# RemyMuj/UnityRayTracer

Measured on AMD Instinct MI355X. Metric: Mrays/sec @1920x1080, 8 bounces, higher is better.
Workload: dtype f32

## Files before the change

### unityraytracer_amd/csrc/context.cpp

```cpp
#include "experiments.h"
#include "context_impl.h"

#include <climits>
#include <limits>
#include <memory>

#include "normals.h"
#include "normals_plan.h"
#include "present.h"
#include "reproject.h"
#include "skin.h"

using namespace urtd;

namespace {

const char* const kBindNames[B_COUNT] = {"_MeshObjects", "_Vertices", "_Indices", "_Normals", "_Spheres", "_MeshBVH", "_SphereBVH"};
const int kBindStride[B_COUNT] = {URT_STRIDE_MESHOBJECT, URT_STRIDE_VEC3, URT_STRIDE_INDEX, URT_STRIDE_VEC3,
                                  URT_STRIDE_SPHERE, URT_STRIDE_BVHNODE, URT_STRIDE_BVHNODE};

std::string g_create_error;

BlasResult g_debug_blas;

// ... 821 lines not shown
  if (!device_src || !hip_stream) return fail(ctx, URT_ERR_INVALID_ARGUMENT, "device_src / hip_stream is NULL");
  Texture* t = find_texture(ctx, texture);
  if (!t) return fail(ctx, URT_ERR_INVALID_HANDLE, "unknown texture handle");
  if (first_group_row < 0 || row_stride < 1) return fail(ctx, URT_ERR_INVALID_ARGUMENT, "bad strip arguments");
  if (ctx->pend.n > 0) {
    bool touched = ctx->pend.tex == texture;
    for (const PostOp& q : ctx->pend.ops) touched = touched || q.touches(texture);
    if (touched) { int rc = flush_pending(ctx); if (rc) return rc; }
  }
  if (in_slab(ctx, *t)) { int rc = detach_from_slab(ctx, *t); if (rc) return rc; }
  int n_strips = strip_count((t->h + 7) / 8, first_group_row, row_stride);
  t->other_writes = true;
  URT_HIP(ctx, hipSetDevice(ctx->device));
  if (rgb) URT_HIP(ctx, launch_pack_rows_rgb(t->dev, (float*)const_cast<void*>(device_src), t->w, t->h, first_group_row, row_stride, n_strips, false,
                                            alpha, (hipStream_t)hip_stream));
  else URT_HIP(ctx, launch_pack_rows(t->dev, (float4*)const_cast<void*>(device_src), t->w, t->h, first_group_row, row_stride, n_strips, false,
                                     (hipStream_t)hip_stream));
  return URT_OK;
}

int urt_texture_unpack_rows_on(urt_context* ctx, urt_handle texture, int first_group_row, int row_stride, const void* device_src,
                               void* hip_stream) {
  return unpack_on_impl(ctx, texture, first_group_row, row_stride, device_src, hip_stream, false, 0.0f);
}

int urt_texture_pack_rows_rgb(urt_context* ctx, urt_handle texture, int first_group_row, int row_stride, void* device_dst,
                              uint64_t* out_bytes) {
  return pack_impl(ctx, texture, first_group_row, row_stride, device_dst, true, out_bytes, true);
}

int urt_texture_unpack_rows_rgb(urt_context* ctx, urt_handle texture, int first_group_row, int row_stride, const void* device_src,
                                float alpha, void* hip_stream) {
  if (ctx && !device_src) return fail(ctx, URT_ERR_INVALID_ARGUMENT, "device_src is NULL");
  if (hip_stream) return unpack_on_impl(ctx, texture, first_group_row, row_stride, device_src, hip_stream, true, alpha);
  return pack_impl(ctx, texture, first_group_row, row_stride, const_cast<void*>(device_src), false, nullptr, true, alpha);
}

int urt_texture_unpack_rows(urt_context* ctx, urt_handle texture, int first_group_row, int row_stride, const void* device_src) {
  if (ctx && !device_src) return fail(ctx, URT_ERR_INVALID_ARGUMENT, "device_src is NULL");
  return pack_impl(ctx, texture, first_group_row, row_stride, const_cast<void*>(device_src), false, nullptr);
}

namespace {
enum : unsigned { kBool = 1, kStale = 2, kFlushAgain = 4, kOnChange = 8 };
struct OptionRow { const char* name; int urt_context::Options::* field; int lo, hi; const char* msg; unsigned flags; bool (*ok)(int); };
using O = urt_context::Options;
const OptionRow kOptions[] = {
  {"blas_builder", &O::blas_builder, -1, 3, "blas_builder must be -1 (auto), 0 (host SAH), 1 (GPU LBVH), 2 (GPU LBVH built top-down within a depth budget) or 3 (binned SAH on the GPU)", kStale | kOnChange, nullptr},
  {"frames_per_launch", &O::frames_per_launch, 0, kMaxFramesPerLaunch, "frames_per_launch must be in [0, 64] (0 = auto)", 0, nullptr},
  {"count_stats", &O::count_stats, INT_MIN, INT_MAX, "", kBool, nullptr},
  {"time_dispatch", &O::time_dispatch, INT_MIN, INT_MAX, "", kBool, nullptr},
  {"kernel_mode", &O::kernel_mode, 0, 5, "kernel_mode must be 0..5", 0, nullptr},
  {"block_threads", &O::block_threads, 64, 256, "block_threads must be 64, 128 or 256", 0, [](int v) { return v == 64 || v == 128 || v == 256; }},
  {"blas_leaf_max", nullptr , 1, 8, "blas_leaf_max must be in [1, 8]", kStale, nullptr},
  {"blas_min", &O::blas_min, 0, 256, "blas_min must be in [0, 256] (0 = auto; kernel_mode 5 counts the waiting rays of a workgroup)", 0, nullptr},
  {"blas_exit", &O::blas_exit, 0, 64, "blas_exit must be in [0, 64] (0 = auto)", 0, nullptr},
  {"refill_min", &O::refill_min, 1, 64, "refill_min must be in [1, 64]", 0, nullptr},
  {"waves_per_cu", &O::waves_per_cu, 0, 32, "waves_per_cu must be in [0, 32] (0 = auto)", 0, nullptr},
  {"sched_block", &O::sched_block, 0, 256, "sched_block must be 0 (auto), 64 or 256", 0, [](int v) { return v == 0 || v == 64 || v == 256; }},
  {"stack_pad", &O::stack_pad, 0, 96, "stack_pad must be in [0, 96]", 0, nullptr},
  {"radiance_persist", &O::radiance_persist, -1, 1, "radiance_persist must be -1 (auto), 0 or 1", 0, nullptr},
  {"shade_min", &O::shade_min, 1, 64, "shade_min must be in [1, 64]", 0, nullptr},
  {"front_list", &O::front_list, -1, 2, "front_list must be -1 (auto), 0, 1 or 2", 0, nullptr},
  {"shade_split", &O::shade_split, -1, 1, "shade_split must be -1 (auto), 0 or 1", 0, nullptr},
  {"serve_refill", &O::serve_refill, 1, 64, "serve_refill must be in [1, 64]", 0, nullptr},
  {"sky_min", &O::sky_min, 1, 64, "sky_min must be in [1, 64]", 0, nullptr},
  {"tile_order", &O::tile_order, -1, 1, "tile_order must be -1 (auto), 0 or 1", 0, nullptr},
  {"lds_tlas", &O::lds_tlas, INT_MIN, INT_MAX, "", kBool, nullptr},
  {"top_front", &O::top_front, -1, 1, "top_front must be -1 (auto), 0 or 1", 0, nullptr},
  {"top_nodes", &O::top_nodes, -1, kTopOrderNodes, "top_nodes must be in [0, 256], or -1 (auto)", 0, nullptr},
  {"pool_k", &O::pool_k, 1, 4, "pool_k must be in [1, 4]", 0, nullptr},
  {"pool_refill", &O::pool_refill, 1, 256, "pool_refill must be in [1, 256]", 0, nullptr},
  {"pool_blas_min", &O::pool_blas_min, 1, 256, "pool_blas_min must be in [1, 256]", 0, nullptr},
  {"pool_blas_exit", &O::pool_blas_exit, 1, 64, "pool_blas_exit must be in [1, 64]", 0, nullptr},
  {"pool_other_min", &O::pool_other_min, 1, 64, "pool_other_min must be in [1, 64]", 0, nullptr},
  {"pool_inloop", &O::pool_inloop, 1, 64, "pool_inloop must be in [1, 64]", 0, nullptr},
  {"frame_group", &O::frame_group, 1, kMaxFramesPerLaunch, "frame_group must be in [1, 64]", 0, nullptr},
  {"work_shards", &O::work_shards, 1, (int)kWorkShards, "work_shards must be a power of two in [1, 64]", 0, [](int v) { return (v & (v - 1)) == 0; }},
  {"qnodes", &O::qnodes, -1, 1, "qnodes must be -1 (auto), 0 or 1", kStale, nullptr},
  {"lbvh_slack", &O::lbvh_slack, 0, 16, "lbvh_slack must be 0..16", kStale | kOnChange, nullptr},
  {"overlap_launches", &O::overlap_launches, 0, 2, "overlap_launches must be 0 (off), 1 (auto) or 2 (always)", kFlushAgain, nullptr},
  {"blas_cones", &O::blas_cones, -1, 1, "blas_cones must be -1 (auto), 0 or 1", kStale | kOnChange, nullptr},
  {"front_cull", &O::front_cull, 0, 1, "front_cull must be 0 or 1", kFlushAgain | kStale | kOnChange, nullptr},
  {"refit", &O::refit, INT_MIN, INT_MAX, "", kBool | kStale, nullptr},
  {"refit_vertices", &O::refit_vertices, INT_MIN, INT_MAX, "", kBool, nullptr},
  {"refit_rebuild_pct", &O::refit_rebuild_pct, 0, INT_MAX, "refit_rebuild_pct must be 0 (never rebuild) or greater than 100", 0, [](int v) { return v == 0 || v > 100; }},
  {"watchdog_cap", &O::watchdog_cap, 0, INT_MAX, "watchdog_cap must be >= 0 (0 = auto)", 0, nullptr},
  {"xcd_run", &O::xcd_run, 0, 4096, "xcd_run must be in [0, 4096] (0 = auto)", 0, nullptr},
};
}

int urt_set_option(urt_context* ctx, const char* name, int value) {
  if (!ctx) return fail(nullptr, URT_ERR_INVALID_ARGUMENT, "ctx is NULL");
  if (!name) return fail(ctx, URT_ERR_INVALID_ARGUMENT, "option name is NULL");
  { (void)hipSetDevice(ctx->device); int rc = flush_pending(ctx); if (rc) return rc; }
  const OptionRow* r = std::find_if(std::begin(kOptions), std::end(kOptions), [&](const OptionRow& o) { return std::strcmp(name, o.name) == 0; });
  if (r == std::end(kOptions)) return fail(ctx, URT_ERR_INVALID_ARGUMENT, std::string("unknown option ") + name);
  if (value < r->lo || value > r->hi || (r->ok && !r->ok(value))) return fail(ctx, URT_ERR_INVALID_ARGUMENT, r->msg);
  if (r->flags & kBool) value = value ? 1 : 0;
  const bool act = !(r->flags & kOnChange) || ctx->opt.*r->field != value;
  if ((r->flags & kFlushAgain) && act) { int rc = flush_pending(ctx); if (rc) return rc; }
  if ((r->flags & kStale) && act) { ctx->scene_dirty = true; ctx->dirty_full = true; }
  if (r->field) ctx->opt.*r->field = value; else set_blas_leaf_max(value);
  return URT_OK;
}

int urt_get_counters(urt_context* ctx, urt_counters* out) {
  if (!ctx) return fail(nullptr, URT_ERR_INVALID_ARGUMENT, "ctx is NULL");
  if (!out) return fail(ctx, URT_ERR_INVALID_ARGUMENT, "out is NULL");
  URT_HIP(ctx, hipSetDevice(ctx->device));
  { int rc = flush_pending(ctx); if (rc) return rc; }
  URT_HIP(ctx, hipStreamSynchronize(touch(ctx)));
  resolve_timing(ctx);
  std::vector<DevCounters> shards(kCounterShards);
  URT_HIP(ctx, hipMemcpy(shards.data(), ctx->d_counters.get(), sizeof(DevCounters) * kCounterShards, hipMemcpyDeviceToHost));
  std::memset(out, 0, sizeof *out);
  for (const DevCounters& dc : shards) {
    out->rays += dc.rays; out->tlas_nodes += dc.tlas_nodes; out->blas_nodes += dc.blas_nodes; out->tri_tests += dc.tri_tests;
    out->sphere_tests += dc.sphere_tests; out->hit_tri += dc.hit_tri; out->hit_sphere += dc.hit_sphere;
    out->hit_ground += dc.hit_ground; out->hit_sky += dc.hit_sky;
    out->watchdog_trips += (uint32_t)dc.watchdog;
  }
  out->pixels = ctx->pixels_dispatched;
  out->dispatches = ctx->dispatches;
  out->launches = ctx->launches;
  out->trace_ms = ctx->trace_ms;
  return URT_OK;
}

int urt_reset_counters(urt_context* ctx) {
  if (!ctx) return fail(nullptr, URT_ERR_INVALID_ARGUMENT, "ctx is NULL");
  URT_HIP(ctx, hipSetDevice(ctx->device));
  { int rc = flush_pending(ctx); if (rc) return rc; }
  URT_HIP(ctx, hipStreamSynchronize(touch(ctx)));
  resolve_timing(ctx);
  URT_HIP(ctx, hipMemset(ctx->d_counters.get(), 0, sizeof(DevCounters) * kCounterShards));
  if (ctx->h_trip_flag) __atomic_store_n(ctx->h_trip_flag.get(), 0u, __ATOMIC_RELEASE);
  ctx->dispatches = 0;
  ctx->launches = 0;
  ctx->pixels_dispatched = 0;
  ctx->trace_ms = 0;
  return URT_OK;
}

#ifdef URT_STAMPS
__attribute__((visibility("default"))) int urt_debug_read_stamps(urt_context* ctx, unsigned long long* out, int n_waves) {
  (void)hipStreamSynchronize(touch(ctx));
  hipError_t e = hipMemcpy(out, (char*)ctx->d_next.get() + urt_context::kStampOffset, (size_t)n_waves * sizeof(unsigned long long), hipMemcpyDeviceToHost);
  (void)hipMemset((char*)ctx->d_next.get() + urt_context::kStampOffset, 0, urt_context::kStampBytes);
  return (int)e;
}
#endif

int urt_debug_serve_stats(urt_context* ctx, unsigned long long* out6) {
  if (!ctx) return fail(nullptr, URT_ERR_INVALID_ARGUMENT, "ctx is NULL");
  if (!out6) return fail(ctx, URT_ERR_INVALID_ARGUMENT, "out6 is NULL");
  URT_HIP(ctx, hipSetDevice(ctx->device));
  { int rc = flush_pending(ctx); if (rc) return rc; }
  URT_HIP(ctx, hipStreamSynchronize(touch(ctx)));
  std::vector<DevCounters> shards(kCounterShards);
  URT_HIP(ctx, hipMemcpy(shards.data(), ctx->d_counters.get(), sizeof(DevCounters) * kCounterShards, hipMemcpyDeviceToHost));
  for (int q = 0; q < 6; q++) out6[q] = 0;
  for (const DevCounters& dc : shards) for (int q = 0; q < 6; q++) out6[q] += dc.serve[q];
  return URT_OK;
}

// ... 172 lines not shown
```

### unityraytracer_amd/csrc/context_impl.h

```cpp
#pragma once
#include <hip/hip_runtime.h>

#include <algorithm>
#include <cmath>
#include <cstdio>
#include <cstring>
#include <new>
#include <string>
#include <unordered_map>
#include <utility>
#include <vector>

#include "../../include/urt.h"
#include "../../include/urt_math.h"
#include "blas_builder.h"
#include "kernels.h"
#include "owned.h"
#include "urt_device.h"

namespace urtd {

struct Buffer {
  int count = 0, stride = 0;
  std::vector<uint8_t> host;
  bool has_data = false;
  int dirty_first = 0, dirty_last = -1;
  void mark_dirty(int first, int last) {
    if (dirty_last < dirty_first) { dirty_first = first; dirty_last = last; }
    else { dirty_first = std::min(dirty_first, first); dirty_last = std::max(dirty_last, last); }
  }
  DeviceBuf<char> mirror;
  int stale_first = 0, stale_last = -1;
  uint64_t downloads = 0;
  bool stale() const { return stale_last >= stale_first; }
  void mark_stale(int first, int last) {
    if (!stale()) { stale_first = first; stale_last = last; }
    else { stale_first = std::min(stale_first, first); stale_last = std::max(stale_last, last); }
  }
};

struct Texture {
  int w = 0, h = 0;
  float4* dev = nullptr;
  float4* own = nullptr;
  DeviceBuf<float4> storage;
  bool external = false;
  bool ptr_exposed = false;
  bool other_writes = false;
  int n_regions = 0;
  int rg[4] = {0, 0, 0, 0};
};

struct DevNormalsPlan {
  urt_handle vertices = 0;
  int n_vertices = 0;
  int first = 0, count = 0, n_lists = 0, n_triangles = 0, n_entries = 0, max_valence = 0;
  DeviceBuf<int32_t> tris, entries, ranges;
  uint64_t device_bytes = 0;
};

enum BindSlot { B_MESHOBJECTS, B_VERTICES, B_INDICES, B_NORMALS, B_SPHERES, B_MESHBVH, B_SPHEREBVH, B_COUNT };

}

struct urt_context {
  urtd::Stream own_stream;
  int device = 0;
  hipStream_t stream = nullptr;
  std::string err;
  std::unordered_map<urt_handle, urtd::Buffer> buffers;
  std::unordered_map<urt_handle, urtd::Texture> textures;
  std::unordered_map<urt_handle, urtd::DevNormalsPlan> normals_plans;
  urt_handle next_id = 1;

  urt_handle bound[urtd::B_COUNT] = {0, 0, 0, 0, 0, 0, 0};
  urt_handle t_sky = 0, t_result = 0;
  float c2w[16] = {0}, invp[16] = {0};
  bool c2w_set = false, invp_set = false;
  float pixel_off[2] = {0, 0};
  float seed = 0;
  int num_bounces = 0, num_rays = 0;

  struct Options {
    int refit = 1;
    int refit_vertices = 1;
    int refit_rebuild_pct = 0;
    int qnodes = 0;
    int count_stats = 0, time_dispatch = 0, kernel_mode = 3;
    int block_threads = 64, xcd_run = 0 , work_shards = 64, frame_group = 64, refill_min = 16, waves_per_cu = 0 , blas_min = 0 , blas_exit = 0 ;
    int pool_k = 2, pool_refill = 32, pool_blas_min = 48, pool_blas_exit = 8, pool_inloop = 16, pool_other_min = 24;
    int sched_block = 0;
    int stack_pad = 0;
    int radiance_persist = -1;
    int shade_min = 32, sky_min = 32;
    int serve_refill = 16;
    int front_list = -1;
    int shade_split = -1;
    int tile_order = -1;
    int lds_tlas = 1;
    int top_front = -1;
    int top_nodes = -1;
    int blas_builder = -1;
    int frames_per_launch = 0;
    int watchdog_cap = 0;
    int lbvh_slack = 6;
    int front_cull = 1;
    int overlap_launches = 1;
    int blas_cones = -1;
  } opt;

  bool scene_dirty = true;
  unsigned int dirty_slots = 0;
  bool dirty_full = true;
  struct Scene {
    urtd::DevScene ds{};
    std::vector<urtd::DeviceBuf<char>> scene_allocs;
    struct RefitAux {
      const float* vertices = nullptr; const int32_t* indices = nullptr;
      const float* normals = nullptr;
      int32_t* renormed = nullptr;
      double* cost_base = nullptr; double* cost_now = nullptr;
      int32_t* parent = nullptr; int32_t* node_mesh = nullptr; int32_t* depth = nullptr;
      float4* cbox = nullptr; unsigned int* ext = nullptr;
      float* matrices = nullptr; int32_t* moved = nullptr;
      bool ready = false;
    } refit;
    float4* qbuf = nullptr;
    float4* cbuf = nullptr;
    float qnode_quality = 0;
    int4* cone_rng[2] = {nullptr, nullptr};
    const int4* cone_ranges = nullptr;
    bool cones_in_use = false;
    const float4* aov_albedo = nullptr;
    size_t cap_materials = 0, cap_mesh_tlas = 0, cap_sphere_tlas = 0, cap_sphere_pr = 0, cap_aov_albedo = 0;
    int32_t* d_mesh_leaf = nullptr;
    size_t cap_mesh_leaf = 0;
    int walk_f4 = 0;
    int n_blas_nodes = 0;
    int n_scene_tris = 0;
    int scene_max_depth = 0;
    int tlas_stack = 2, blas_stack = 2;
    unsigned int watchdog_steps = 1u << 16;
    std::vector<int32_t> h_mesh_root, h_small_first;
    std::vector<int32_t> h_vert_lo, h_vert_hi;
    int n_vertices = 0, n_normals = 0;
    std::vector<float> h_cost_base;
    std::vector<uint8_t> prev_mesh_objects;
  } scene;
  uint64_t scene_epoch = 0;
  float last_prepare_ms = 0;
  int last_builder = 0;
  uint64_t refitted_meshes = 0, incremental_preps = 0;
  uint64_t deformed_meshes = 0, renormed_meshes = 0, deform_bytes = 0, forced_rebuilds = 0;
  float last_cost_ratio = 0;
  urtd::BlasCache blas_cache;
  int sched_groups = 0;
  urtd::DeviceBuf<float4> zero_sky;

  urtd::PathQueues q{};
  urtd::DeviceBuf<float4> q_store[2][4];
  urtd::DeviceBuf<unsigned int> q_counts;

  urtd::DeviceBuf<urtd::DevCounters> d_counters;
  static constexpr size_t kStampOffset = urtd::kWorkShards * 128, kStampBytes = 65536 * 16 * sizeof(unsigned long long), kWorkCounterBytes = kStampOffset + kStampBytes;
  urtd::DeviceBuf<unsigned int> d_next;
  urtd::DeviceBuf<float4> d_mail;
  static constexpr int kTableSlots = 4;
  urtd::PinnedBuf<urtd::FrameUniforms> h_tables; urtd::DeviceBuf<urtd::FrameUniforms> d_tables;
  urtd::Event table_ev[kTableSlots];
  unsigned int table_next = 0;
  uint64_t pixels_dispatched = 0;
  int n_cus = 256;

  uint64_t dispatches = 0;
  std::vector<std::pair<urtd::Event, urtd::Event>> timing;
  float trace_ms = 0;

  enum class OpKind { BlendAdd, BlendHistory, Copy, PackRows };
  struct PostOp {
    OpKind kind;
// ... 140 lines not shown
```

### unityraytracer_amd/csrc/frame_batch.cpp

```cpp
#include "experiments.h"
#include "context_impl.h"

#include "reproject.h"

namespace urtd {

static unsigned int sched_trip_cap(urt_context* ctx, const FrameParams& P, int n_frames) {
  if (ctx->opt.watchdog_cap > 0) return (unsigned int)ctx->opt.watchdog_cap;
  uint64_t per = std::max<uint64_t>(1, (uint64_t)std::max(1, P.num_rays) * (uint64_t)std::max(1, P.num_bounces) / 8u);
  uint64_t cap = (1ull << 24) * (uint64_t)std::max(1, n_frames) * per;
  return (unsigned int)std::min<uint64_t>(cap, 0xfffffff0ull);
}

static int ensure_queues(urt_context* ctx, size_t n_paths, size_t n_counts) {
  for (int k = 0; k < 8; k++) {
    if (int rc = reserve(ctx, ctx->q_store[k / 4][k % 4], n_paths, "path queue allocation", touch(ctx))) return rc;
    ctx->q.s[k / 4][k % 4] = ctx->q_store[k / 4][k % 4].get();
  }
  if (int rc = reserve(ctx, ctx->q_counts, n_counts, "path queue allocation", touch(ctx))) return rc;
  ctx->q.counts = ctx->q_counts.get();
  return URT_OK;
}

int resolve_timing(urt_context* ctx) {
// ... 336 lines not shown
    if (ctx->stream != ctx->own_stream.get()) return 1;
    uint64_t frame_bytes = (uint64_t)P.width * (uint64_t)P.height * sizeof(float4);
    lim = (int)std::min<uint64_t>(kAutoFrames, std::max<uint64_t>(1, (8ull << 30) / std::max<uint64_t>(1, frame_bytes)));
  }
  uint64_t slots = std::max<uint64_t>(1, ((uint64_t)P.tiles_x * (uint64_t)P.n_strips + (uint64_t)std::max(64, ctx->opt.xcd_run)) * 64u);
  lim = (int)std::min<uint64_t>((uint64_t)lim, std::max<uint64_t>(1, 0xfffffffeull / slots / 2));
  return std::max(1, std::min(lim, (int)kMaxFramesPerLaunch));
}

int bind_sky(urt_context* ctx, DevScene& S) {
  Texture* sky = find_texture(ctx, ctx->t_sky);
  if (sky) { S.sky = sky->dev; S.sky_w = sky->w; S.sky_h = sky->h; }
  else {
    if (!ctx->zero_sky) {
      URT_HIP(ctx, ctx->zero_sky.alloc(1));
      URT_HIP(ctx, hipMemsetAsync(ctx->zero_sky.get(), 0, sizeof(float4), touch(ctx)));
    }
    S.sky = ctx->zero_sky.get(); S.sky_w = 1; S.sky_h = 1;
  }
  return URT_OK;
}

int do_dispatch(urt_context* ctx, int kernel, int gx, int gy, int gz, int first_row, int row_stride) {
  if (kernel != 0) return fail(ctx, URT_ERR_INVALID_ARGUMENT, "kernel index must be 0 (CSMain)");
  if (gx < 0 || gy < 0 || gz < 0 || first_row < 0 || row_stride < 1)
    return fail(ctx, URT_ERR_INVALID_ARGUMENT, "negative thread-group count or bad strip arguments");
  urt_handle res_h = ctx->t_result;
  Texture* res = find_texture(ctx, res_h);
  if (!res) return fail(ctx, URT_ERR_UNBOUND, "Dispatch: no texture bound to \"Result\" (RM:803)");
  if (res->w > 65535 || res->h > 65535) return fail(ctx, URT_ERR_INVALID_ARGUMENT, "Result larger than 65535 pixels per side");
  URT_HIP(ctx, hipSetDevice(ctx->device));
  if (int rc = current_scene(ctx)) return rc;
  ctx->dispatches++;
  if (gx == 0 || gy == 0 || gz == 0) return URT_OK;

  DevScene S = ctx->scene.ds;
  { int rc = bind_sky(ctx, S); if (rc) return rc; }

  FrameParams P{};
  std::memcpy(P.c2w, ctx->c2w, sizeof P.c2w);
  std::memcpy(P.invp, ctx->invp, sizeof P.invp);
  P.pixel_off_x = ctx->pixel_off[0]; P.pixel_off_y = ctx->pixel_off[1];
  P.seed = ctx->seed;
  P.num_bounces = ctx->num_bounces; P.num_rays = ctx->num_rays;
  P.width = res->w; P.height = res->h;
  long rw = std::min<long>((long)gx * 8, res->w), rh = std::min<long>((long)gy * 8, res->h);
  P.region_w = (int)rw; P.region_h = (int)rh;
  P.tiles_x = (P.region_w + 7) / 8;
  P.first_group_row = first_row; P.row_stride = row_stride;
  P.n_strips = strip_count((P.region_h + 7) / 8, first_row, row_stride);
  P.tlas_stack = lane_stack_size(ctx).tlas; P.blas_stack = lane_stack_size(ctx).blas; P.watchdog_steps = ctx->scene.watchdog_steps;
  P.block_threads = ctx->opt.block_threads; P.xcd_run = ctx->opt.xcd_run; P.tile_order = ctx->opt.tile_order >= 0 ? ctx->opt.tile_order : (S.n_meshes == 0 ? 1 : 0); P.refill_min = ctx->opt.refill_min;
  P.blas_min = ctx->opt.blas_min > 0 ? ctx->opt.blas_min : (S.n_meshes > 1 ? 24 : 16);
  P.blas_exit = ctx->opt.blas_exit > 0 ? ctx->opt.blas_exit : (S.n_meshes > 1 ? 9 : 14); P.shade_min = ctx->opt.shade_min; P.sky_min = ctx->opt.sky_min;
  P.n_frames = 1; P.frame_stride = 0;
  P.sched_trips = sched_trip_cap(ctx, P, 1); P.trip_flag = ctx->d_trip_flag;
  if (P.n_strips == 0 || P.tiles_x == 0) return URT_OK;
  P.n_shards = ctx->opt.work_shards; P.frame_group = ctx->opt.frame_group;
  if (ctx->opt.xcd_run <= 0) P.xcd_run = ctx->opt.kernel_mode >= 2 ? auto_run_length(P, 1) : 1;
  if ((uint64_t)P.tiles_x * (uint64_t)P.n_strips * 64u >= 0xffffffffull)
    return fail(ctx, URT_ERR_INVALID_ARGUMENT, "Dispatch: too many pixel slots in one dispatch");

  {
    uint64_t px = 0;
    for (int j = 0; j < P.n_strips; j++) {
      int y0 = (first_row + j * row_stride) * 8;
      px += (uint64_t)std::max(0, std::min(P.region_h - y0, 8)) * (uint64_t)P.region_w;
    }
    ctx->pixels_dispatched += px;
  }
  bool degenerate = P.num_bounces <= 0 || P.num_rays <= 0;
  int mode = degenerate ? 0 : ctx->opt.kernel_mode;
  if ((mode == 3 || mode == 5) && P.num_bounces >= (1 << 24)) mode = 2;
  bool count = ctx->opt.count_stats != 0;
  const int region[4] = {P.region_w, P.region_h, first_row, row_stride};
  const bool full_cover = P.region_w == res->w && P.region_h == res->h && first_row == 0 && row_stride == 1;

  if (mode == 3 || mode == 5) {
    bool top_in_front = ctx->opt.top_front < 0 ? S.n_meshes > 1 : ctx->opt.top_front != 0;
    P.serve = mode == 5 && ctx->scene.n_blas_nodes > 0;
    P.pool_inloop = ctx->opt.serve_refill;
    int front_mode = configure_sched(ctx, S, P, top_in_front);
    P.shade_split = ctx->opt.shade_split != 0;
    const FrameUniforms fu = bound_camera(ctx);
    bool same_region = res->n_regions == 1 && std::memcmp(res->rg, region, sizeof region) == 0;
    bool renamable = !res->external && !res->ptr_exposed && (full_cover || (!res->other_writes && (res->n_regions == 0 || same_region)));
    int limit = renamable ? batch_limit(ctx, P) : 1;
    urt_context::Pending& B = ctx->pend;
    if (B.n > 0) {
      const FrameParams& Q = B.P;
      bool same = B.tex == res_h && B.scene_epoch == ctx->scene_epoch && B.S.sky == S.sky && B.S.sky_w == S.sky_w && B.S.sky_h == S.sky_h &&
                  B.count == count && B.front_mode == front_mode && Q.serve == P.serve && Q.num_bounces == P.num_bounces && Q.num_rays == P.num_rays &&
                  Q.width == P.width && Q.height == P.height && Q.region_w == P.region_w && Q.region_h == P.region_h &&
                  Q.first_group_row == P.first_group_row && Q.row_stride == P.row_stride && B.n < B.limit && limit > 1;
      if (!same) { int rc = flush_pending(ctx); if (rc) return rc; }
    }
    if (limit > 1 && B.n == 0) {
      int rc = ensure_slab(ctx, res_h, *res, limit); if (rc) return rc;
      if (!ctx->slab || ctx->slab_tex != res_h || ctx->slab_frames < 2) limit = 1;
    }
    if (B.n == 0) { int rc = bind_sky(ctx, S); if (rc) return rc; }
    if (limit <= 1) {
      FrameTable T{};
      T.f[0] = fu;
      P.frame_group = 1;
      int rc = launch_sched_frames(ctx, S, P, T, res->dev, front_mode, count);
      if (rc) return rc;
    } else {
      if (B.n == 0) {
        B.limit = std::min(limit, ctx->slab_frames);
        B.tex = res_h; B.scene_epoch = ctx->scene_epoch; B.S = S; B.P = P; B.front_mode = front_mode; B.count = count;
      }
      B.T.f[B.n] = fu;
      res->dev = ctx->slab.get() + (size_t)B.n * ctx->slab_stride;
      B.n++;
    }
  } else {
    int rc = flush_pending(ctx); if (rc) return rc;
    int nb = 0, k = 0;
    if (mode == 1) {
      size_t n_paths = (size_t)P.tiles_x * 64 * (size_t)P.n_strips;
      rc = ensure_queues(ctx, n_paths, (size_t)P.num_rays * (size_t)(P.num_bounces + 1));
      if (rc) return rc;
    } else if (mode == 2) {
      int waves_per_block = P.block_threads / 64;
      long want = ((long)P.tiles_x * P.n_strips + waves_per_block - 1) / waves_per_block;
      int wpc = ctx->opt.waves_per_cu;
      if (wpc <= 0) wpc = 20;
      long resident = (long)ctx->n_cus * wpc / waves_per_block;
      nb = (int)std::max(1L, std::min(want, resident));
    } else if (mode == 4) {
      P.block_threads = 64;
      P.refill_min = ctx->opt.pool_refill; P.blas_min = ctx->opt.pool_blas_min; P.blas_exit = ctx->opt.pool_blas_exit;
      P.pool_inloop = ctx->opt.pool_inloop; P.pool_other_min = ctx->opt.pool_other_min;
      k = ctx->opt.pool_k;
      size_t lds = pool_lds_bytes(P, k);
      while (k > 1 && lds > 160 * 1024) { k--; lds = pool_lds_bytes(P, k); }
      if (lds > 160 * 1024) return fail(ctx, URT_ERR_OUT_OF_MEMORY, "kernel_mode 4: the scene's traversal stacks do not fit the LDS of one CU; use kernel_mode 3");
      int fit = (int)std::max<size_t>(1, (160 * 1024) / lds);
      int wpc = ctx->opt.waves_per_cu > 0 ? ctx->opt.waves_per_cu : fit;
      long want = ((long)P.tiles_x * P.n_strips * 64 + 64L * k - 1) / (64L * k);
      nb = (int)std::max(1L, std::min(want, (long)ctx->n_cus * wpc));
    }
    const hipStream_t st = touch(ctx);
    rc = timed_launch(ctx, st, mode, 0, P, count, ctx->opt.waves_per_cu, [&](TraceLaunchRecord* rec) {
      switch (mode) {
        case 1: return launch_wavefront(S, P, ctx->q, res->dev, ctx->d_counters.get(), count, st, rec);
        case 2: return launch_persist(S, P, res->dev, ctx->d_counters.get(), ctx->d_next.get(), nb, count, st, rec);
        case 4: return launch_pool(S, P, res->dev, ctx->d_counters.get(), ctx->d_next.get(), nb, k, count, st, rec);
        default: return launch_mega(S, P, res->dev, ctx->d_counters.get(), count, st, rec);
      }
    });
    if (rc) return rc;
  }
  if (res->n_regions == 0) { res->n_regions = 1; std::memcpy(res->rg, region, sizeof region); }
  else if (std::memcmp(res->rg, region, sizeof region) != 0) res->n_regions = 2;
  return URT_OK;
}

}
```

### unityraytracer_amd/csrc/front_device.h

```cpp
#pragma once
#include "frame_device.h"

namespace {

struct FrontLds {
  const float4* mesh_tlas = nullptr;
  const int32_t* mesh_root = nullptr;
  const float4* sphere_tlas = nullptr;
  const float4* sphere_pr = nullptr;
  const float4* small_tris = nullptr;
  const int32_t* small_first = nullptr;
};

template <bool COUNT, bool TOPF = false, bool RAYS = true, int SP0 = 0, bool CONES = false>
__device__ __forceinline__ bool trace_front(const DevScene& S, bool fresh, v3 o, v3 d, HitRec& best, int& check, bool& seen,
                                            int* tl, int stride, int32_t& cur, LocalCounters& lc, const FrontLds& L = FrontLds(),
                                            const float4* top = nullptr, int top_nodes = 0, int* bl = nullptr, int* sp_out = nullptr) {
  if (fresh) {
    if (RAYS) lc.rays++;
    best.t = URT_INF; best.kid = 0; best.u = 0; best.v = 0;
    float t = -o.y / d.y;
    if (t > 0 && t < best.t) { best.t = t; best.kid = 1; }
    check = 0; seen = false;
    if (S.n_meshes > 0) { check = 1; tl[0] = 0; }
  }
  v3 rcp = mk3(1.0f / (d.x + kEPSILON), 1.0f / (d.y + kEPSILON), 1.0f / (d.z + kEPSILON));
  const bool may_cull = S.cull_any != 0;
  while (check > 0) {
    check--;
    int bi = tl[check * stride];
    bool hit = false; int index = -1;
    float t_min = 0.0f, t_max = 0.0f; int cull_word = 0;
    if (bi < S.n_mesh_tlas) {
      if (COUNT) lc.tlas_nodes++;
      float4 a, b;
      if (L.mesh_tlas) { a = L.mesh_tlas[2 * bi]; b = L.mesh_tlas[2 * bi + 1]; } else { a = S.mesh_tlas[2 * bi]; b = S.mesh_tlas[2 * bi + 1]; }
      index = as_int(a.w);
      if (may_cull) { hit = tlas_slab_t(a, b, o, rcp, t_min, t_max); cull_word = as_int(b.w); }
      else hit = tlas_slab(a, b, o, rcp);
    }
    if (hit) {
      if (index < 0) { tl[check * stride] = bi * 2 + 1; check++; tl[check * stride] = bi * 2 + 2; check++; }
      else seen = true;
    }
    bool culled = false;
    if (cull_word != 0) { float t = -o.y / d.y; culled = tlas_cull(t_min, t_max, t > 0 ? t : URT_INF); }
    if (seen && !culled && index >= 0 && index < S.n_meshes) {
      int32_t root;
      if (L.mesh_root) root = L.mesh_root[index]; else root = S.mesh_root[index];
      if (root < 0 && root != kBlasDone) {
        int bi_local = -1;
        if (L.small_tris) test_leaf<COUNT>(S, root, o, d, best, bi_local, lc, L.small_tris, L.small_first[index]);
        else test_leaf<COUNT>(S, root, o, d, best, bi_local, lc);
      } else if (root != kEmptyMeshRoot) {
        if (TOPF) {
          int sp = SP0;
          if (root < top_nodes) {
            BlasRay R = blas_ray(o, d);
            if (SP0 == 1) root = blas_walk_top_ptr<COUNT, CONES>(top, top_nodes, root, R, best.t, bl, sp, lc, CONES ? cone_ray_word(d) : 0);
            else do root = blas_node_step_top<COUNT>(top, root, R, best.t, bl, sp, lc); while (root >= 0 && root < top_nodes);
          }
          *sp_out = sp;
          if (root == kBlasDone) continue;
        }
        cur = root;
        return true;
      }
    }
  }
  if (S.n_spheres > 0) {
    int c2 = 1; tl[0] = 0; bool seen2 = false;
    while (c2 > 0) {
      c2--;
      int bi = tl[c2 * stride];
      bool hit = false; int index = -1;
      if (bi < S.n_sphere_tlas) {
        if (COUNT) lc.tlas_nodes++;
        float4 a, b;
        if (L.sphere_tlas) { a = L.sphere_tlas[2 * bi]; b = L.sphere_tlas[2 * bi + 1]; } else { a = S.sphere_tlas[2 * bi]; b = S.sphere_tlas[2 * bi + 1]; }
        index = as_int(a.w);
        hit = tlas_slab(a, b, o, rcp);
      }
      if (hit) {
        if (index < 0) { tl[c2 * stride] = bi * 2 + 1; c2++; tl[c2 * stride] = bi * 2 + 2; c2++; }
        else seen2 = true;
      }
      if (seen2 && index >= 0 && index < S.n_spheres) intersect_sphere<COUNT>(S, index, o, d, best, lc, L.sphere_pr);
    }
  }
  return false;
}

__device__ __forceinline__ int list_get(const int* tl, int j) {
  unsigned int w = (unsigned int)tl[j >= 6 ? 64 : 0];
  return (int)((w >> (5 * (j >= 6 ? j - 6 : j))) & 31u);
}

#ifdef URT_STAMPS
#define URT_FS_DECL , unsigned long long* fs
#define URT_FS_ARG , fs_arr
#define URT_FS(stmt) stmt
#else
#define URT_FS_DECL
#define URT_FS_ARG
#define URT_FS(stmt)
#endif
template <bool COUNT, int SP0 = 0, bool CONES = false>
__device__ __forceinline__ int front_listed(const DevScene& S, const FrameParams& P, bool mine, bool fresh, v3 o, v3 d, HitRec& best, int& cs,
                                            int* tl, int32_t& cur, LocalCounters& lc, const FrontLds& L, const float4* top, int* bl, int& sp,
                                            unsigned int& wave_rays URT_FS_DECL) {
  URT_FS(unsigned long long fs_t0 = wall_clock64();)
  int remaining = cs & 0xff, cursor = cs >> 8;
  const int n_fresh = __popcll(wballot(mine && fresh)), n_resumed = __popcll(wballot(mine && !fresh));
  const bool walk_now = n_fresh >= 16 || n_resumed == 0;
  if (!walk_now) mine = mine && !fresh;
  else wave_rays += (unsigned int)n_fresh;
  const bool put_off = !walk_now && fresh;
  if (mine && fresh) {
    best.t = URT_INF; best.kid = 0; best.u = 0; best.v = 0;
    float t = -o.y / d.y;
    if (t > 0 && t < best.t) { best.t = t; best.kid = 1; }
    v3 rcp = mk3(1.0f / (d.x + kEPSILON), 1.0f / (d.y + kEPSILON), 1.0f / (d.z + kEPSILON));
    int count = 0, check = 0;
    unsigned int l0 = 0, l1 = 0;
    bool seen = false;
    if (S.n_meshes > 0) { check = 1; tl[0] = 0; }
    const float t_ground = best.t;
    while (check > 0) {
      check--;
      int bi = tl[check * 64];
      bool hit = false, culled = false; int index = -1;
      if (bi < S.n_mesh_tlas) {
        if (COUNT) lc.tlas_nodes++;
        float4 a = L.mesh_tlas[2 * bi], b = L.mesh_tlas[2 * bi + 1];
        index = as_int(a.w);
        float t_min, t_max;
        hit = tlas_slab_t(a, b, o, rcp, t_min, t_max);
        culled = leaf_culled(b, t_min, t_max, t_ground);
      }
      if (hit) {
        if (index < 0) { tl[check * 64] = bi * 2 + 1; check++; tl[check * 64] = bi * 2 + 2; check++; }
        else seen = true;
      }
      if (seen && !culled && index >= 0 && index < S.n_meshes && L.mesh_root[index] != kEmptyMeshRoot) {
        if (count < 6) l0 |= (unsigned int)index << (5 * count); else l1 |= (unsigned int)index << (5 * (count - 6));
        count++;
      }
    }
    tl[0] = (int)l0; tl[64] = (int)l1;
    remaining = count; cursor = 0;
  }
  URT_FS(if (walk_now && n_fresh > 0) { fs[0] += wall_clock64() - fs_t0; fs[3]++; fs[6] += (unsigned long long)n_fresh; })
  bool need = false;
  bool has = mine && remaining > 0;
  for (;;) {
    int obj = 0; int32_t root = kEmptyMeshRoot;
    URT_FS(unsigned long long fs_t1 = wall_clock64();)
    for (;;) {
      if (has) { obj = list_get(tl, cursor); root = L.mesh_root[obj]; }
      bool small = has && root < 0;
      if (wballot(small) == 0) break;
      URT_FS(fs[4]++;)
      if (small) {
        int bi_local = -1;
        if (L.small_tris) test_leaf<COUNT>(S, root, o, d, best, bi_local, lc, L.small_tris, L.small_first[obj]);
        else test_leaf<COUNT>(S, root, o, d, best, bi_local, lc);
        cursor++; remaining--; has = remaining > 0;
      }
    }
    URT_FS(fs[1] += wall_clock64() - fs_t1; fs_t1 = wall_clock64();)
// ... 166 lines not shown
```

### unityraytracer_amd/csrc/kernels.hip

```cpp
#include "experiments.h"
#include "front_device.h"
#include "launch_host.h"
#include <utility>

namespace {

#ifndef URT_SCHED_OCC
#define URT_SCHED_OCC 5
#endif
template <bool COUNT, int BLOCK, int FMODE, bool MULTI, bool QN = false>
__global__ __launch_bounds__(BLOCK, URT_SCHED_OCC) void k_sched(DevScene S, FrameParams P, const FrameUniforms* __restrict__ T, float4* __restrict__ result, DevCounters* ctr,
                                               unsigned int* __restrict__ next) {
  constexpr bool CONES = !COUNT && !QN;
  extern __shared__ int lds[];
  float4* lds4 = (float4*)lds;
  const float4* top = lds4;
  for (int i = threadIdx.x; i < P.top_nodes * 4; i += blockDim.x) lds4[i] = S.blas_cnodes[i];
  int at = P.top_nodes * 4;
  FrontLds L;
  if (P.lds_mesh) {
    for (int i = threadIdx.x; i < 2 * S.n_mesh_tlas; i += blockDim.x) lds4[at + i] = S.mesh_tlas[i];
    L.mesh_tlas = lds4 + at; at += 2 * S.n_mesh_tlas;
    for (int i = threadIdx.x; i < S.n_meshes; i += blockDim.x) ((int32_t*)(lds4 + at))[i] = S.mesh_root[i];
    L.mesh_root = (const int32_t*)(lds4 + at); at += (S.n_meshes + 3) / 4;
    if (P.lds_small) {
      for (int i = threadIdx.x; i < S.n_meshes; i += blockDim.x) ((int32_t*)(lds4 + at))[i] = S.mesh_small_first[i];
      L.small_first = (const int32_t*)(lds4 + at); at += (S.n_meshes + 3) / 4;
      for (int m = threadIdx.x; m < S.n_meshes; m += blockDim.x) {
        int sf = S.mesh_small_first[m];
        if (sf >= 0) {
          uint32_t code = ~(uint32_t)S.mesh_root[m];
          uint32_t first = code >> 3, cnt = (code & 7u) + 1u;
          for (uint32_t q = 0; q < 3 * cnt; q++) lds4[at + 3 * sf + q] = S.tri_verts[3 * (size_t)first + q];
        }
      }
      L.small_tris = lds4 + at; at += 3 * S.n_small;
    }
  }
  WalkLds W;
  if (FMODE == 3) {
    const float4* wsrc = S.mesh_tlas + 2 * S.n_mesh_tlas;
    for (int i = threadIdx.x; i < P.walk_f4; i += blockDim.x) lds4[at + i] = wsrc[i];
    W.hdr = (const int*)(lds4 + at); W.pos_tab = W.hdr + 16; W.eval = lds4 + at + 20; at += P.walk_f4;
    if (P.lds_small) {
      for (int m = threadIdx.x; m < S.n_meshes; m += blockDim.x) {
        int sf = S.mesh_small_first[m];
        if (sf >= 0) {
          uint32_t code = ~(uint32_t)S.mesh_root[m];
          uint32_t first = code >> 3, cnt = (code & 7u) + 1u;
          for (uint32_t q = 0; q < 3 * cnt; q++) lds4[at + 3 * sf + q] = S.tri_verts[3 * (size_t)first + q];
        }
      }
      L.small_tris = lds4 + at; at += 3 * S.n_small;
    }
  }
  if (P.lds_sphere) {
    for (int i = threadIdx.x; i < 2 * S.n_sphere_tlas; i += blockDim.x) lds4[at + i] = S.sphere_tlas[i];
    L.sphere_tlas = lds4 + at; at += 2 * S.n_sphere_tlas;
    for (int i = threadIdx.x; i < S.n_spheres; i += blockDim.x) lds4[at + i] = S.sphere_pr[i];
    L.sphere_pr = lds4 + at; at += S.n_spheres;
  }
  __syncthreads();
  int* tl = lds + at * 4 + (threadIdx.x >> 6) * ((P.tlas_stack + P.blas_stack) * 64) + (threadIdx.x & 63);
  int* bl = tl + P.tlas_stack * 64;
  LocalCounters lc;
  unsigned int tiles_per_frame;
  const unsigned int ntiles = launch_tiles(P, tiles_per_frame);
  WorkCursor wc; wc.shard = blockIdx.x & ((unsigned int)P.n_shards - 1u);
  bool exhausted = false;
  int st = ST_DEAD;
  int xy = 0;
  int ray_i = 0, kf = 0;
  float seed = 0;
  v3 o = mk3(0, 0, 0), d = mk3(0, 0, 1), energy = mk3(0, 0, 0), res = mk3(0, 0, 0), avg = mk3(0, 0, 0);
  HitRec best; best.t = URT_INF; best.kid = 0; best.u = 0; best.v = 0;
  int cs = 0;
  bl[0] = kBlasDone;
  int32_t cur = kBlasDone; int sp = 1, best_i = -1;
  unsigned int wave_iters = 0, wave_rays = 0;
  bool watchdog = false;
#ifdef URT_STAMPS
  unsigned long long ph_t[4] = {0, 0, 0, 0}, ph_lanes[4] = {0, 0, 0, 0}, ph_trips[4] = {0, 0, 0, 0};
  unsigned long long t_begin = wall_clock64(), t_dry = 0;
  unsigned long long c_begin = __builtin_amdgcn_s_memtime();
  unsigned long long dr_trips[4] = {0, 0, 0, 0}, dr_t[3] = {0, 0, 0}, dr_live = 0, dr_lanes3 = 0;
  unsigned long long fs_arr[7] = {0, 0, 0, 0, 0, 0, 0};
  unsigned long long rf_t[3] = {0, 0, 0};
  unsigned long long bl_part[3] = {0, 0, 0};
#endif

  for (;;) {
    if (watchdog) break;
#ifdef URT_STAMPS
    if (exhausted && !t_dry) t_dry = wall_clock64();
#endif
    unsigned long long mD = wballot(st == ST_DEAD);
    int nD = __popcll(mD);
    int nB = __popcll(wballot(st == ST_BLAS));
    int nS = __popcll(wballot(st == ST_SHADE));
    int nK = __popcll(wballot(st == ST_SKY));
    int nF = __popcll(wballot(st == ST_FRONT || st == ST_RESUME));
    if (!exhausted && nD > 0 && (nD >= P.refill_min || nB + nS + nK + nF == 0)) {
      int x = 0, y = 0, frame = 0;
#ifdef URT_STAMPS
      unsigned long long t_rf = wall_clock64();
#endif
      bool got = wave_fetch_pixels(P, mD, st == ST_DEAD, next, ntiles, wc, exhausted, x, y, tiles_per_frame, &frame);
#ifdef URT_STAMPS
      rf_t[0] += wall_clock64() - t_rf; t_rf = wall_clock64();
#endif
      for_each_frame(got, frame, [&](int f, bool mine) {
        if (mine) {
          st = ST_FRONT;
          ray_i = 0; kf = frame << 24; xy = x | (y << 16);
          avg = mk3(0, 0, 0); res = mk3(0, 0, 0); energy = mk3(1, 1, 1);
          camera_ray_frame(T, f, P, x, y, true, seed, o, d);
        }
      });
#ifdef URT_STAMPS
      rf_t[1] += wall_clock64() - t_rf; rf_t[2]++;
#endif
      nF = __popcll(wballot(st == ST_FRONT || st == ST_RESUME));
      nD = __popcll(wballot(st == ST_DEAD));
    }
    bool can_refill = !exhausted && nD >= P.refill_min;
    if (++wave_iters > P.sched_trips) { watchdog = true; break; }
    int phase;
    int exit_below = 1;
    bool sky_too = false;
    if (nB >= P.blas_min) { phase = ST_BLAS; if (nS + nK + nF > 0 || can_refill) exit_below = min(P.blas_exit, nB); }
    else if (P.shade_split) {
      if (nS >= P.shade_min) phase = ST_SHADE;
      else if (nK >= P.sky_min) phase = ST_SKY;
      else if (nF > 0) phase = ST_FRONT;
      else if (nS > 0 && nS >= nK) phase = ST_SHADE;
      else if (nK > 0) phase = ST_SKY;
      else if (nB > 0) phase = ST_BLAS;
      else if (exhausted) break;
      else continue;
    }
    else if (nS + nK >= P.shade_min) { phase = nS > 0 ? ST_SHADE : ST_SKY; sky_too = true; }
    else if (nF > 0) phase = ST_FRONT;
    else if (nS + nK > 0) { phase = nS > 0 ? ST_SHADE : ST_SKY; sky_too = true; }
    else if (nB > 0) phase = ST_BLAS;
    else if (exhausted) break;
    else continue;

#ifdef URT_STAMPS
    unsigned long long t_ph = wall_clock64();
    int ph_id = phase == ST_FRONT ? 0 : phase == ST_BLAS ? 1 : 2;
    ph_lanes[ph_id] += (unsigned long long)(phase == ST_FRONT ? nF : phase == ST_BLAS ? nB : phase == ST_SHADE ? nS : nK);
    ph_trips[ph_id]++;
    if (exhausted) { if (!dr_live) dr_live = 64 - nD; dr_trips[ph_id]++; }
#endif
    if (phase == ST_FRONT) {
      if (FMODE < 2) wave_rays += (unsigned int)__popcll(wballot(st == ST_FRONT));
      if (FMODE >= 2) {
        bool mine = st == ST_FRONT || st == ST_RESUME;
        int r = FMODE == 3 ? front_masked<COUNT, 1, CONES>(S, P, mine, st == ST_FRONT, o, d, best, cs, tl, cur, lc, L, W, top, bl, sp, wave_rays URT_FS_ARG)
                           : front_listed<COUNT, 1, CONES>(S, P, mine, st == ST_FRONT, o, d, best, cs, tl, cur, lc, L, top, bl, sp, wave_rays URT_FS_ARG);
        if (mine && r != 2) {
          if (r == 1) { best_i = -1; st = ST_BLAS; }
          else st = best.t < URT_INF ? ST_SHADE : ST_SKY;
        }
      } else if (st == ST_FRONT || st == ST_RESUME) {
        sp = 1;
        int check = cs & 0xff; bool seen = (cs >> 8) != 0;
        bool need = FMODE == 1 ? trace_front<COUNT, true, false, 1, CONES>(S, st == ST_FRONT, o, d, best, check, seen, tl, 64, cur, lc, L, top, P.top_nodes, bl, &sp)
                               : trace_front<COUNT, false, false, 1>(S, st == ST_FRONT, o, d, best, check, seen, tl, 64, cur, lc, L);
        cs = check | (seen ? 256 : 0);
        if (need) { best_i = -1; st = ST_BLAS; }
        else st = best.t < URT_INF ? ST_SHADE : ST_SKY;
      }
    } else if (phase == ST_BLAS) {
      bool mine = st == ST_BLAS;
      BlasRay R = blas_ray(o, d);
      int* spp = bl + (sp - 1) * 64;
      const int rw = CONES ? cone_ray_word(d) : 0;
      if (mine && cur >= 0 && cur < P.top_nodes) {
        do {
          if (COUNT) lc.blas_nodes++;
          const float4* n = top + 4 * cur;
          cur = CONES ? blas_node_eval_cone_ptr(n[0], n[1], n[2], n[3], R, best.t, rw, spp) : blas_node_eval_ptr(n[0], n[1], n[2], n[3], R, best.t, spp);
        } while (cur >= 0 && cur < P.top_nodes);
      }
      int32_t c = mine ? cur : kBlasDone;
      int budget = __builtin_amdgcn_readfirstlane((int)min(P.watchdog_steps, 0x7fffffffu));
      const int exit_s = __builtin_amdgcn_readfirstlane(exit_below);
      QRay Q;
      if (QN) Q = make_qray(o, d, S.blas_qnodes[0], S.blas_qnodes[1]);
      for (;;) {
        int nA = __popcll(wballot(c != kBlasDone));
        if (nA < exit_s) break;
        if (--budget < 0) { watchdog = true; break; }
#ifdef URT_STAMPS
        ph_trips[3]++; ph_lanes[3] += (unsigned long long)nA;
        if (exhausted) { dr_trips[3]++; dr_lanes3 += (unsigned long long)nA; }
#endif
        int nI = __popcll(wballot(c >= 0));
        bool node_trip = 2 * nI >= nA;
#ifdef URT_STAMPS
        bl_part[0] += (unsigned long long)(node_trip ? nI : nA - nI); bl_part[1] += node_trip ? 1 : 0; bl_part[2] += (unsigned long long)(node_trip ? nA - nI : 0);
#endif
        if (node_trip) {
          if (QN) {
            if (c >= 0) {
              const float4* n = (const float4*)((const char*)(S.blas_qnodes + 2) + ((uint32_t)c << 5));
              float4 u0 = n[0], u1 = n[1];
              c = qnode_eval_ptr(u0, u1, Q, best.t, spp);
            }
          } else if (c >= 0) {
            if (COUNT) lc.blas_nodes++;
            const float4* n = (const float4*)((const char*)S.blas_cnodes + ((uint32_t)c << 6));
            float4 q0 = n[0], q1 = n[1], q2 = n[2], q3 = n[3];
            c = CONES ? blas_node_eval_cone_ptr(q0, q1, q2, q3, R, best.t, rw, spp) : blas_node_eval_ptr(q0, q1, q2, q3, R, best.t, spp);
          }
        } else if (c < 0 && c != kBlasDone) {
          test_leaf<COUNT>(S, c, o, d, best, best_i, lc);
          c = *spp; spp -= 64;
        }
      }
      if (mine) { cur = c; sp = ((int)(spp - bl) >> 6) + 1; }
      if (mine && cur == kBlasDone) st = ((FMODE == 3 ? cs : (cs & 0xff)) == 0 && S.n_spheres == 0) ? (best.t < URT_INF ? ST_SHADE : ST_SKY) : ST_RESUME;
    } else {
      bool next_ray = false;
      bool cont = false, shaded = false;
      if (phase == ST_SHADE) {
        if (st == ST_SHADE) { shaded = true; cont = shade_surface<COUNT>(S, best, o, d, energy, res, seed, (float)(xy & 0xffff), (float)((unsigned)xy >> 16), lc); }
      }
      if (phase == ST_SKY || (sky_too && nK > 0)) {
        if (st == ST_SKY) { shaded = true; cont = shade_sky<COUNT>(S, d, energy, res, lc); }
      }
      if (shaded) {
        kf++;
        st = ST_FRONT;
        if (!cont || (kf & 0xffffff) >= P.num_bounces) {
          v3 sum = (MULTI ? avg : mk3(0, 0, 0)) + res;
          if (MULTI) { avg = sum; ray_i++; next_ray = ray_i < P.num_rays; }
          if (!next_ray) {
            float n = (float)P.num_rays;
            st_nt(result + (size_t)((unsigned)kf >> 24) * P.frame_stride + (size_t)((unsigned)xy >> 16) * P.width + (xy & 0xffff),
                      MULTI ? make_float4(sum.x / n, sum.y / n, sum.z / n, 1.0f) : make_float4(sum.x, sum.y, sum.z, 1.0f));
            st = ST_DEAD;
          }
        }
      }
      if (MULTI) {
        for_each_frame(next_ray, (int)((unsigned)kf >> 24), [&](int f, bool mine) {
          if (mine) {
            res = mk3(0, 0, 0); energy = mk3(1, 1, 1); kf &= (int)0xff000000;
            camera_ray_frame(T, f, P, xy & 0xffff, (int)((unsigned)xy >> 16), false, seed, o, d);
          }
        });
// ... 183 lines not shown
```

### unityraytracer_amd/csrc/urt_device.h

```cpp
#pragma once
#include <stdint.h>
#include <hip/hip_runtime.h>

#include "blas_builder.h"

namespace urtd {

struct DevScene {
  const float4* mesh_tlas;   int n_mesh_tlas;
  const float4* sphere_tlas; int n_sphere_tlas;
  const float4* sphere_pr;   int n_spheres;
  const float4* materials;
  const int32_t* mesh_root;  int n_meshes;
  const int32_t* mesh_small_first; int n_small;
  const float4* blas_nodes;
  const float4* blas_cnodes;
  const float4* blas_qnodes;
  const float4* tri_verts;
  const float4* tri_norms;
  const float4* sky;         int sky_w, sky_h;
  int cull_any;
};

struct FrameParams {
  float c2w[16];
  float invp[16];
  float pixel_off_x, pixel_off_y;
  float seed;
  int num_bounces;
  int num_rays;
  int width, height;
  int region_w, region_h;
  int tiles_x;
  int first_group_row;
  int row_stride;
  int n_strips;
  int tlas_stack;
  int blas_stack;
  int block_threads;
  int tile_order;
  int xcd_run;
  int n_shards;
  int frame_group;
  int refill_min;
  int blas_min;
  int shade_min;
  int sky_min;
  int shade_split;
  int blas_exit;
  int top_nodes;
  int lds_small;
  int lds_mesh, lds_sphere;
  int walk_f4;
  int serve;
  int pool_inloop;
  int pool_other_min;
  unsigned int watchdog_steps;
  unsigned int sched_trips;
  unsigned int* trip_flag;
  int n_frames;
  unsigned int frame_stride;
};

struct FrameUniforms {
  float c2w[16];
  float invp[16];
  float pixel_off_x, pixel_off_y;
  float seed;
  float pad;
};
static constexpr int kMaxFramesPerLaunch = 64;
struct FrameTable { FrameUniforms f[kMaxFramesPerLaunch]; };

struct LaneStackSize { int tlas, blas; };

static constexpr unsigned int kWorkShards = 64;
static constexpr int kCounterShards = 256;
struct alignas(128) DevCounters {
  unsigned long long rays, tlas_nodes, blas_nodes, tri_tests, sphere_tests;
  unsigned long long hit_tri, hit_sphere, hit_ground, hit_sky;
  unsigned long long watchdog;
  unsigned long long serve[6];
};
static_assert(sizeof(DevCounters) == 128, "one counter shard = one 128-byte line");

struct PathQueues {
  float4* s[2][4];
  unsigned int* counts;
};

}
```

Baseline: 19400.

## Prioritize fresh front pass and add single-TLAS fast front path

Adds a front_fuse option (auto by default) that, in wavefront modes below 2, checks first for freshly spawned ST_FRONT lanes and runs a front phase for them before computing the other state ballots. For scenes with a single mesh TLAS node and no spheres, it uses a specialised front_single routine that tests the ground plane and the one TLAS box directly instead of the generic TLAS walk. It also skips several per-iteration ballots in the lower modes. One risk: front_fuse shares a union slot with pool_other_min in FrameParams, so the two could clobber each other.

```diff
diff --git a/unityraytracer_amd/csrc/context.cpp b/unityraytracer_amd/csrc/context.cpp
--- a/unityraytracer_amd/csrc/context.cpp
+++ b/unityraytracer_amd/csrc/context.cpp
@@ -927,6 +927,7 @@
   {"overlap_launches", &O::overlap_launches, 0, 2, "overlap_launches must be 0 (off), 1 (auto) or 2 (always)", kFlushAgain, nullptr},
   {"blas_cones", &O::blas_cones, -1, 1, "blas_cones must be -1 (auto), 0 or 1", kStale | kOnChange, nullptr},
   {"front_cull", &O::front_cull, 0, 1, "front_cull must be 0 or 1", kFlushAgain | kStale | kOnChange, nullptr},
+  {"front_fuse", &O::front_fuse, -1, 1, "front_fuse must be -1 (auto), 0 or 1", kOnChange, nullptr},
   {"refit", &O::refit, INT_MIN, INT_MAX, "", kBool | kStale, nullptr},
   {"refit_vertices", &O::refit_vertices, INT_MIN, INT_MAX, "", kBool, nullptr},
   {"refit_rebuild_pct", &O::refit_rebuild_pct, 0, INT_MAX, "refit_rebuild_pct must be 0 (never rebuild) or greater than 100", 0, [](int v) { return v == 0 || v > 100; }},
diff --git a/unityraytracer_amd/csrc/context_impl.h b/unityraytracer_amd/csrc/context_impl.h
--- a/unityraytracer_amd/csrc/context_impl.h
+++ b/unityraytracer_amd/csrc/context_impl.h
@@ -96,6 +96,7 @@
     int serve_refill = 16;
     int front_list = -1;
     int shade_split = -1;
+    int front_fuse = -1;
     int tile_order = -1;
     int lds_tlas = 1;
     int top_front = -1;
diff --git a/unityraytracer_amd/csrc/frame_batch.cpp b/unityraytracer_amd/csrc/frame_batch.cpp
--- a/unityraytracer_amd/csrc/frame_batch.cpp
+++ b/unityraytracer_amd/csrc/frame_batch.cpp
@@ -442,6 +442,7 @@
     P.pool_inloop = ctx->opt.serve_refill;
     int front_mode = configure_sched(ctx, S, P, top_in_front);
     P.shade_split = ctx->opt.shade_split != 0;
+    P.front_fuse = ctx->opt.front_fuse == 0 ? 0 : (S.n_mesh_tlas == 1 && S.n_meshes > 0 && S.n_spheres == 0 ? 2 : 1);
     const FrameUniforms fu = bound_camera(ctx);
     bool same_region = res->n_regions == 1 && std::memcmp(res->rg, region, sizeof region) == 0;
     bool renamable = !res->external && !res->ptr_exposed && (full_cover || (!res->other_writes && (res->n_regions == 0 || same_region)));
diff --git a/unityraytracer_amd/csrc/front_device.h b/unityraytracer_amd/csrc/front_device.h
--- a/unityraytracer_amd/csrc/front_device.h
+++ b/unityraytracer_amd/csrc/front_device.h
@@ -86,6 +86,38 @@
         else seen2 = true;
       }
       if (seen2 && index >= 0 && index < S.n_spheres) intersect_sphere<COUNT>(S, index, o, d, best, lc, L.sphere_pr);
+    }
+  }
+  return false;
+}
+
+template <bool COUNT>
+__device__ __forceinline__ bool front_single(const DevScene& S, v3 o, v3 d, HitRec& best, int& cs, int32_t& cur, LocalCounters& lc, const FrontLds& L) {
+  best.t = URT_INF; best.kid = 0; best.u = 0; best.v = 0;
+  float t = -o.y / d.y;
+  if (t > 0 && t < best.t) { best.t = t; best.kid = 1; }
+  v3 rcp = mk3(1.0f / (d.x + kEPSILON), 1.0f / (d.y + kEPSILON), 1.0f / (d.z + kEPSILON));
+  if (COUNT) lc.tlas_nodes++;
+  float4 a, b;
+  if (L.mesh_tlas) { a = L.mesh_tlas[0]; b = L.mesh_tlas[1]; } else { a = S.mesh_tlas[0]; b = S.mesh_tlas[1]; }
+  const int index = as_int(a.w);
+  bool hit; float t_min = 0.0f, t_max = 0.0f; int cull_word = 0;
+  if (S.cull_any != 0) { hit = tlas_slab_t(a, b, o, rcp, t_min, t_max); cull_word = as_int(b.w); }
+  else hit = tlas_slab(a, b, o, rcp);
+  const bool seen = hit && index >= 0;
+  cs = seen ? 256 : 0;
+  bool culled = false;
+  if (cull_word != 0) culled = tlas_cull(t_min, t_max, t > 0 ? t : URT_INF);
+  if (seen && !culled && index < S.n_meshes) {
+    int32_t root;
+    if (L.mesh_root) root = L.mesh_root[index]; else root = S.mesh_root[index];
+    if (root < 0 && root != kBlasDone) {
+      int bi_local = -1;
+      if (L.small_tris) test_leaf<COUNT>(S, root, o, d, best, bi_local, lc, L.small_tris, L.small_first[index]);
+      else test_leaf<COUNT>(S, root, o, d, best, bi_local, lc);
+    } else if (root != kEmptyMeshRoot) {
+      cur = root;
+      return true;
     }
   }
   return false;
diff --git a/unityraytracer_amd/csrc/kernels.hip b/unityraytracer_amd/csrc/kernels.hip
--- a/unityraytracer_amd/csrc/kernels.hip
+++ b/unityraytracer_amd/csrc/kernels.hip
@@ -96,11 +96,14 @@
 #endif
     unsigned long long mD = wballot(st == ST_DEAD);
     int nD = __popcll(mD);
-    int nB = __popcll(wballot(st == ST_BLAS));
-    int nS = __popcll(wballot(st == ST_SHADE));
-    int nK = __popcll(wballot(st == ST_SKY));
-    int nF = __popcll(wballot(st == ST_FRONT || st == ST_RESUME));
-    if (!exhausted && nD > 0 && (nD >= P.refill_min || nB + nS + nK + nF == 0)) {
+    int nB = 0, nS = 0, nK = 0, nF = 0;
+    if (FMODE >= 2) {
+      nB = __popcll(wballot(st == ST_BLAS));
+      nS = __popcll(wballot(st == ST_SHADE));
+      nK = __popcll(wballot(st == ST_SKY));
+      nF = __popcll(wballot(st == ST_FRONT || st == ST_RESUME));
+    }
+    if (!exhausted && nD > 0 && (nD >= P.refill_min || (FMODE < 2 ? nD == 64 : nB + nS + nK + nF == 0))) {
       int x = 0, y = 0, frame = 0;
 #ifdef URT_STAMPS
       unsigned long long t_rf = wall_clock64();
@@ -120,15 +123,29 @@
 #ifdef URT_STAMPS
       rf_t[1] += wall_clock64() - t_rf; rf_t[2]++;
 #endif
-      nF = __popcll(wballot(st == ST_FRONT || st == ST_RESUME));
-      nD = __popcll(wballot(st == ST_DEAD));
+      if (FMODE >= 2) {
+        nF = __popcll(wballot(st == ST_FRONT || st == ST_RESUME));
+        nD = __popcll(wballot(st == ST_DEAD));
+      }
+    }
+    bool fresh_pass = false;
+    if constexpr (FMODE < 2) {
+      if (P.front_fuse) { nF = __popcll(wballot(st == ST_FRONT)); fresh_pass = nF > 0; }
+      if (!fresh_pass) {
+        nB = __popcll(wballot(st == ST_BLAS));
+        nS = __popcll(wballot(st == ST_SHADE));
+        nK = __popcll(wballot(st == ST_SKY));
+        nF = __popcll(wballot(st == ST_FRONT || st == ST_RESUME));
+        nD = 64 - (nB + nS + nK + nF);
+      }
     }
     bool can_refill = !exhausted && nD >= P.refill_min;
     if (++wave_iters > P.sched_trips) { watchdog = true; break; }
     int phase;
     int exit_below = 1;
     bool sky_too = false;
-    if (nB >= P.blas_min) { phase = ST_BLAS; if (nS + nK + nF > 0 || can_refill) exit_below = min(P.blas_exit, nB); }
+    if (fresh_pass) phase = ST_FRONT;
+    else if (nB >= P.blas_min) { phase = ST_BLAS; if (nS + nK + nF > 0 || can_refill) exit_below = min(P.blas_exit, nB); }
     else if (P.shade_split) {
       if (nS >= P.shade_min) phase = ST_SHADE;
       else if (nK >= P.sky_min) phase = ST_SKY;
@@ -163,12 +180,16 @@
           if (r == 1) { best_i = -1; st = ST_BLAS; }
           else st = best.t < URT_INF ? ST_SHADE : ST_SKY;
         }
-      } else if (st == ST_FRONT || st == ST_RESUME) {
+      } else if (st == ST_FRONT || (!fresh_pass && st == ST_RESUME)) {
         sp = 1;
-        int check = cs & 0xff; bool seen = (cs >> 8) != 0;
-        bool need = FMODE == 1 ? trace_front<COUNT, true, false, 1, CONES>(S, st == ST_FRONT, o, d, best, check, seen, tl, 64, cur, lc, L, top, P.top_nodes, bl, &sp)
-                               : trace_front<COUNT, false, false, 1>(S, st == ST_FRONT, o, d, best, check, seen, tl, 64, cur, lc, L);
-        cs = check | (seen ? 256 : 0);
+        bool need;
+        if (FMODE == 0 && fresh_pass && P.front_fuse == 2) need = front_single<COUNT>(S, o, d, best, cs, cur, lc, L);
+        else {
+          int check = cs & 0xff; bool seen = (cs >> 8) != 0;
+          need = FMODE == 1 ? trace_front<COUNT, true, false, 1, CONES>(S, st == ST_FRONT, o, d, best, check, seen, tl, 64, cur, lc, L, top, P.top_nodes, bl, &sp)
+                            : trace_front<COUNT, false, false, 1>(S, st == ST_FRONT, o, d, best, check, seen, tl, 64, cur, lc, L);
+          cs = check | (seen ? 256 : 0);
+        }
         if (need) { best_i = -1; st = ST_BLAS; }
         else st = best.t < URT_INF ? ST_SHADE : ST_SKY;
       }
diff --git a/unityraytracer_amd/csrc/urt_device.h b/unityraytracer_amd/csrc/urt_device.h
--- a/unityraytracer_amd/csrc/urt_device.h
+++ b/unityraytracer_amd/csrc/urt_device.h
@@ -54,7 +54,10 @@
   int walk_f4;
   int serve;
   int pool_inloop;
-  int pool_other_min;
+  union {
+    int pool_other_min;
+    int front_fuse;
+  };
   unsigned int watchdog_steps;
   unsigned int sched_trips;
   unsigned int* trip_flag;
```

Result: faster. 19820, median of 6 (+2.1%).
